# google/compare_gan

Hardware: NVIDIA H100
Metric: images/sec G+D step (resnet_cifar10) (higher is better)
Workload: dtype tf32

## Files before the change

### compare_gan_b200/_lib.py

```python
import ctypes
import os
import re

HERE = os.path.dirname(os.path.abspath(__file__))
HEADER = os.path.join(HERE, "..", "include", "cgan_b200.h")
SO_PATH = os.path.join(HERE, "csrc", "libcgan_b200.so")


class ConvDesc(ctypes.Structure):
  _fields_ = [(n, ctypes.c_int32) for n in
              ("n", "h", "w", "cin", "cout", "kh", "kw", "stride", "upsample", "oh", "ow", "pad_t", "pad_l")]


class ConvEpilogue(ctypes.Structure):
  _fields_ = [("bias", ctypes.c_void_p), ("residual", ctypes.c_void_p), ("mask", ctypes.c_void_p),
              ("mask_leak", ctypes.c_float), ("flags", ctypes.c_int32), ("ldy", ctypes.c_int32)]


CONV_RELU, CONV_ROUND_OUT, CONV_IN_TF32, CONV_IN2_TF32 = 1, 2, 4, 8
ACT_ROUND_TF32 = 0x100
OPT_TC_MT, OPT_LAST_PATH, OPT_TC_HALO, OPT_TC_THIN = 1, 2, 3, 6
OPT_LAST_TC_BN, OPT_LAST_TC_MT, OPT_LAST_TC_HALO, OPT_LAST_TC_CTAS_PER_SM, OPT_LAST_TC_EP_SMEM = 7, 8, 9, 10, 11
PATH_NAMES = {0: "simt_fp32", 1: "tcgen05_tf32", 2: "thin_fp32"}

_SCALARS = {"int": ctypes.c_int, "int32_t": ctypes.c_int32, "int64_t": ctypes.c_int64,
            "float": ctypes.c_float, "double": ctypes.c_double, "size_t": ctypes.c_size_t, "uint64_t": ctypes.c_uint64}


def parse_header(path=HEADER):
  src = open(path).read()
  src = re.sub(r"/\*.*?\*/", " ", src, flags=re.S)
  src = re.sub(r"//[^\n]*", " ", src)
  protos = {}
  for m in re.finditer(r"(const\s+char\s*\*|int64_t|int)\s+(cgan_\w+)\s*\(([^;{]*)\)\s*;", src):
    ret, name, args = m.group(1), m.group(2), m.group(3)
    restype = ctypes.c_char_p if "char" in ret else (ctypes.c_int64 if ret == "int64_t" else ctypes.c_int)
    argtypes = []
    args = args.strip()
    if args and args != "void":
      for a in args.split(","):
        a = a.strip()
        if "*" in a:
          argtypes.append(ctypes.c_void_p)
        else:
          ty = a.replace("const", "").split()[0]
          argtypes.append(_SCALARS[ty])
    protos[name] = (restype, argtypes)
  return protos


class CganError(RuntimeError):
  pass


_DLL = {}
# ... 65 lines not shown
```

### compare_gan_b200/csrc/common.cuh

```cuda
#pragma once
#include <cuda_runtime.h>
#include <stdint.h>
#include <stdio.h>
#include <string.h>

#include "../../include/cgan_b200.h"

struct cgan_ctx {
  int device;
  cudaStream_t stream;
  void* ws;
  size_t ws_bytes;
  int math_mode;
  int64_t launches;
  int num_sms;
  int tc_mt_max;
  int tc_halo;
  int tc_thin;
  int last_path;
  int last_tc_bn, last_tc_mt, last_tc_halo;
  int last_tc_ctas_per_sm;
  int last_tc_ep_smem;
  unsigned* counters;
  void* p2p;
  char err[512];
};

constexpr int CGAN_NUM_COUNTERS = 1 << 18;

static inline int cgan_fail(cgan_ctx* ctx, int code, const char* fmt, const char* a = "", const char* b = "") {
  if (ctx) snprintf(ctx->err, sizeof(ctx->err), fmt, a, b);
  return code;
}

#define CGAN_REQUIRE(ctx, cond, msg)                                              \
  do {                                                                            \
    if (!(cond)) return cgan_fail((ctx), CGAN_ERR_ARG, "%s: %s", __func__, msg);  \
  } while (0)

#define CGAN_CUDA(ctx, call)                                                                        \
  do {                                                                                              \
    cudaError_t e__ = (call);                                                                       \
    if (e__ != cudaSuccess) return cgan_fail((ctx), CGAN_ERR_CUDA, "%s: %s", __func__, cudaGetErrorString(e__)); \
  } while (0)

#define CGAN_LAUNCHED(ctx)                                                                          \
  do {                                                                                              \
    (ctx)->launches++;                                                                              \
    cudaError_t e__ = cudaGetLastError();                                                           \
    if (e__ != cudaSuccess) return cgan_fail((ctx), CGAN_ERR_CUDA, "%s: launch: %s", __func__, cudaGetErrorString(e__)); \
  } while (0)

static inline int cgan_ws(cgan_ctx* ctx, size_t bytes, void** out) {
  if (bytes > ctx->ws_bytes) {
    cudaStreamCaptureStatus st = cudaStreamCaptureStatusNone;
// ... 222 lines not shown
```

### compare_gan_b200/csrc/conv_tc.cu

```cuda
#include "tc_common.cuh"

namespace {

using namespace tc;

constexpr int TC_BM = 128;
constexpr int TC_BK = 32;
constexpr int TC_MAX_STAGES = 4;
constexpr int TC_MAX_TAPS = 32;
constexpr int TC_CWARPS = 8;
constexpr int TC_THREADS = 32 * TC_CWARPS + 32;
constexpr int TC_A_BYTES = TC_BM * TC_BK * 4;
constexpr int TC_WG_A_BYTES = TC_A_BYTES / 2;
constexpr int TC_ACC_COLS = 256;

struct TcParams {
  int ntaps, kchunks;
  int off_h[TC_MAX_TAPS], off_w[TC_MAX_TAPS], wtap[TC_MAX_TAPS], amap[TC_MAX_TAPS];
  int bw, bh, bni;
  int tiles_w, tiles_h;
  int rows_used;
  int img_n;
  int relu;
  int vec2;
  int round_a;
  int round_out;
  float mask_leak;
  const float* residual;
  const float* mask;
  int wimg_stride;
  int bn;
  int stages;
  int mt;
  int tiles_total;
  int cout;
  long long s_n, s_h, s_w, base;
  float* out;
  const float* bias;
  int nphases;
  int ph_tap0[5];
  long long ph_base[4];
  int ph_h[4], ph_w[4];
  int hg, hnv;
  int h_off_w[4], h_off_h0[4], h_wtap[4][4];
  int a_halo_bytes;
  int a_box_bytes;
  int sa_stages, sb_stages;
  int ep_smem;
};

struct AMaps { CUtensorMap m[4]; };


__device__ __forceinline__ void tc_tile_origin(const TcParams& p, int t, int& ow0, int& oh0, int& n0) {
  const int tw = t % p.tiles_w; t /= p.tiles_w;
  const int th = t % p.tiles_h;
  const int tn = t / p.tiles_h;
  ow0 = tw * p.bw; oh0 = th * p.bh; n0 = tn * p.bni;
}

__device__ __forceinline__ float epilogue_one(const TcParams& p, float v, int col, long long off) {
  if (p.bias) v += p.bias[col];
  if (p.residual) v += p.residual[off];
  if (p.relu) v = fmaxf(v, 0.f);
  if (p.mask) v = p.mask[off] > 0.f ? v : p.mask_leak * v;
  if (p.round_out) v = rna_tf32(v);
  return v;
}

template <int BN>
__device__ __forceinline__ void tile_epilogue(const TcParams& p, const float* acc, int tile, int nb0, int wg, int warp, int lane,
                                            long long out_base) {
  int ow0, oh0, n0;
  tc_tile_origin(p, tile, ow0, oh0, n0);
  const int c2 = (lane & 3) * 2;
#pragma unroll
  for (int h = 0; h < 2; ++h) {
    const int m = wg * 64 + (warp & 3) * 16 + (lane >> 2) + h * 8;
    const int wi = m % p.bw;
    const int hi = (m / p.bw) % p.bh;
    const int ni = m / (p.bw * p.bh);
    if (!(m < p.rows_used && n0 + ni < p.img_n && oh0 + hi < p.ph_h[blockIdx.z] && ow0 + wi < p.ph_w[blockIdx.z])) continue;
    const long long roff = out_base + (long long)(n0 + ni) * p.s_n + (long long)(oh0 + hi) * p.s_h +
                           (long long)(ow0 + wi) * p.s_w + nb0;
#pragma unroll
    for (int j = 0; j < BN / 8; ++j) {
      const int c = j * 8 + c2;
      if (nb0 + c >= p.cout) continue;
      float2 v = make_float2(acc[4 * j + 2 * h], acc[4 * j + 2 * h + 1]);
      const long long off = roff + c;
      if (p.vec2) {
        if (p.bias) { const float2 b = *reinterpret_cast<const float2*>(p.bias + nb0 + c); v.x += b.x; v.y += b.y; }
        if (p.residual) { const float2 r = *reinterpret_cast<const float2*>(p.residual + off); v.x += r.x; v.y += r.y; }
        if (p.relu) { v.x = fmaxf(v.x, 0.f); v.y = fmaxf(v.y, 0.f); }
        if (p.mask) {
          const float2 mv = *reinterpret_cast<const float2*>(p.mask + off);
          v.x = mv.x > 0.f ? v.x : p.mask_leak * v.x; v.y = mv.y > 0.f ? v.y : p.mask_leak * v.y;
        }
        if (p.round_out) { v.x = rna_tf32(v.x); v.y = rna_tf32(v.y); }
        *reinterpret_cast<float2*>(p.out + off) = v;
      } else {
        p.out[off] = epilogue_one(p, v.x, nb0 + c, off);
        if (nb0 + c + 1 < p.cout) p.out[off + 1] = epilogue_one(p, v.y, nb0 + c + 1, off + 1);
      }
    }
  }
}

template <int BN>
__device__ __forceinline__ void tile_epilogue_smem(const TcParams& p, const float* acc, int tile, int nb0, int wg, int warp,
                                                 int lane, long long out_base, const uint8_t* smem, int stage_bytes,
                                                 uint64_t* full_bar, uint64_t* empty_bar, int& stage, uint32_t& phase,
                                                 int& chunk, int chunks, const float* s_bias) {
  int ow0, oh0, n0;
  tc_tile_origin(p, tile, ow0, oh0, n0);
  const int c2 = (lane & 3) * 2;
  bool ok[2];
  long long roff[2];
  int m[2];
#pragma unroll
  for (int h = 0; h < 2; ++h) {
    m[h] = wg * 64 + (warp & 3) * 16 + (lane >> 2) + h * 8;
    const int wi = m[h] % p.bw;
    const int hi = (m[h] / p.bw) % p.bh;
    const int ni = m[h] / (p.bw * p.bh);
    ok[h] = m[h] < p.rows_used && n0 + ni < p.img_n && oh0 + hi < p.ph_h[blockIdx.z] && ow0 + wi < p.ph_w[blockIdx.z];
    roff[h] = out_base + (long long)(n0 + ni) * p.s_n + (long long)(oh0 + hi) * p.s_h + (long long)(ow0 + wi) * p.s_w + nb0;
  }
  const uint32_t bias_addr = smem_u32(s_bias);
#pragma unroll
  for (int cc = 0; cc < BN / 32; ++cc) {
    mbar_wait(&full_bar[stage], phase);
    const uint32_t e_addr = smem_u32(smem + stage * stage_bytes);
#pragma unroll
    for (int jj = 0; jj < 4; ++jj) {
      const int j = cc * 4 + jj, c = j * 8 + c2;
      if (nb0 + c >= p.cout) continue;
      const float2 b = p.bias ? lds64(bias_addr + c * 4) : make_float2(0.f, 0.f);
#pragma unroll
      for (int h = 0; h < 2; ++h) {
        if (!ok[h]) continue;
        float2 v = make_float2(acc[4 * j + 2 * h], acc[4 * j + 2 * h + 1]);
        const float2 e = lds64(e_addr + sw128_offset(m[h], jj * 8 + c2));
        if (p.bias) { v.x += b.x; v.y += b.y; }
        if (p.residual) { v.x += e.x; v.y += e.y; }
        if (p.relu) { v.x = fmaxf(v.x, 0.f); v.y = fmaxf(v.y, 0.f); }
        if (p.mask) { v.x = e.x > 0.f ? v.x : p.mask_leak * v.x; v.y = e.y > 0.f ? v.y : p.mask_leak * v.y; }
        if (p.round_out) { v.x = rna_tf32(v.x); v.y = rna_tf32(v.y); }
        *reinterpret_cast<float2*>(p.out + roff[h] + c) = v;
      }
    }
    if (chunk + p.stages < chunks) {
      fence_proxy_async();
      named_bar(1 + wg, 128);
      if ((threadIdx.x & 127) == 0) mbar_arrive(&empty_bar[stage]);
    }
    ++chunk;
    if (++stage == p.stages) { stage = 0; phase ^= 1; }
  }
}

constexpr int tc_min_ctas(int bn, int mt) { return bn * mt <= 128 ? 2 : 1; }

__device__ __forceinline__ void tc_round_smem(uint32_t base, int bytes, int q, int nthreads) {
#pragma unroll 4
  for (int i = q * 16; i < bytes; i += nthreads * 16) {
    float4 v = lds128(base + i);
    v.x = rna_tf32(v.x); v.y = rna_tf32(v.y); v.z = rna_tf32(v.z); v.w = rna_tf32(v.w);
    sts128(base + i, v);
  }
}

template <int BN, int MT>
__global__ void __launch_bounds__(TC_THREADS, tc_min_ctas(BN, MT))
conv_tc_kernel(const __grid_constant__ AMaps tm_as, const __grid_constant__ CUtensorMap tm_b, const TcParams p,
               const __grid_constant__ AMaps tm_e) {
  extern __shared__ __align__(1024) uint8_t smem_raw[];
  uint8_t* smem = reinterpret_cast<uint8_t*>((reinterpret_cast<uintptr_t>(smem_raw) + 1023) & ~uintptr_t(1023));
  constexpr int b_bytes = BN * TC_BK * 4;
  constexpr int a_bytes = MT * TC_A_BYTES;
  constexpr int stage_bytes = a_bytes + b_bytes;
  uint64_t* full_bar = reinterpret_cast<uint64_t*>(smem + p.stages * stage_bytes);
  uint64_t* empty_bar = full_bar + p.stages;
  float* s_bias = reinterpret_cast<float*>(smem + p.stages * stage_bytes + 256);

  const int warp = threadIdx.x >> 5, lane = threadIdx.x & 31;
  const int tap0 = p.ph_tap0[blockIdx.z];
  const int num_kb = (p.ph_tap0[blockIdx.z + 1] - tap0) * p.kchunks;

  const int tile0 = blockIdx.x * MT;
  const int nt_here = max(0, min(MT, p.tiles_total - tile0));
  const int nb0 = blockIdx.y * BN;

  if (threadIdx.x == 0) {
    for (int s = 0; s < p.stages; ++s) {
      mbar_init(&full_bar[s], 1);
      mbar_init(&empty_bar[s], 2);
    }
    asm volatile("fence.mbarrier_init.release.cluster;" ::: "memory");
  }
  __syncthreads();

  if (warp == TC_CWARPS) {
    if (lane == 0) {
      asm volatile("prefetch.tensormap [%0];" ::"l"(&tm_as.m[0]) : "memory");
      asm volatile("prefetch.tensormap [%0];" ::"l"(&tm_b) : "memory");
      int stage = 0;
      uint32_t phase = 0;
      for (int kb = 0; kb < num_kb; ++kb) {
        const int tl = kb / p.kchunks, kc = kb - tl * p.kchunks, tap = tap0 + tl;
        mbar_wait(&empty_bar[stage], phase ^ 1);
        uint8_t* sa = smem + stage * stage_bytes;
        uint8_t* sb = sa + a_bytes;
        mbar_expect_tx(&full_bar[stage], (uint32_t)(nt_here * p.rows_used * TC_BK * 4 + b_bytes));
        int ow0, oh0, n0;
        for (int i = 0; i < nt_here; ++i) {
          tc_tile_origin(p, tile0 + i, ow0, oh0, n0);
          tma_load_4d(sa + i * TC_A_BYTES, &tm_as.m[p.amap[tap]], &full_bar[stage], kc * TC_BK, ow0 + p.off_w[tap],
                      oh0 + p.off_h[tap], n0);
        }
        tc_tile_origin(p, tile0, ow0, oh0, n0);
        tma_load_3d(sb, &tm_b, &full_bar[stage], kc * TC_BK, nb0, p.wtap[tap] + n0 * p.wimg_stride);
        if (++stage == p.stages) { stage = 0; phase ^= 1; }
      }
      if (p.ep_smem) {
        const CUtensorMap* em = &tm_e.m[blockIdx.z];
        for (int t = 0; t < nt_here; ++t) {
          int ow0, oh0, n0;
          tc_tile_origin(p, tile0 + t, ow0, oh0, n0);
          for (int cc = 0; cc < BN / 32; ++cc) {
            mbar_wait(&empty_bar[stage], phase ^ 1);
            mbar_expect_tx(&full_bar[stage], (uint32_t)(p.rows_used * TC_BK * 4));
            tma_load_4d(smem + stage * stage_bytes, em, &full_bar[stage], nb0 + cc * 32, ow0, oh0, n0);
            if (++stage == p.stages) { stage = 0; phase ^= 1; }
          }
        }
      }
    }
  } else {
    const int wg = warp >> 2;
    const int q = threadIdx.x & 127;
    if (p.ep_smem && p.bias)
      for (int i = threadIdx.x; i < BN; i += 32 * TC_CWARPS) s_bias[i] = nb0 + i < p.cout ? p.bias[nb0 + i] : 0.f;
    float acc[MT][BN / 2];
#pragma unroll
    for (int t = 0; t < MT; ++t)
#pragma unroll
      for (int i = 0; i < BN / 2; ++i) acc[t][i] = 0.f;
    int stage = 0, prev = -1;
    uint32_t phase = 0;
    for (int kb = 0; kb < num_kb; ++kb) {
      mbar_wait(&full_bar[stage], phase);
      const uint32_t a_addr = smem_u32(smem + stage * stage_bytes) + wg * TC_WG_A_BYTES;
      const uint32_t b_addr = smem_u32(smem + stage * stage_bytes) + a_bytes;
      if (p.round_a) {
        for (int tl = 0; tl < nt_here; ++tl) tc_round_smem(a_addr + tl * TC_A_BYTES, TC_WG_A_BYTES, q, 128);
        fence_proxy_async();
        named_bar(1 + wg, 128);
      }
#pragma unroll
      for (int t = 0; t < MT; ++t)
#pragma unroll
        for (int i = 0; i < BN / 2; ++i) acc_fence(acc[t][i]);
      wgmma_fence();
#pragma unroll
      for (int t = 0; t < MT; ++t) {
#pragma unroll
        for (int k = 0; k < TC_BK / 8; ++k)
          wgmma_tf32<BN>(acc[t], make_desc(a_addr + t * TC_A_BYTES + k * 32), make_desc(b_addr + k * 32));
      }
      wgmma_commit();
      wgmma_wait<1>();
#pragma unroll
      for (int t = 0; t < MT; ++t)
#pragma unroll
        for (int i = 0; i < BN / 2; ++i) acc_fence(acc[t][i]);
      if (prev >= 0 && q == 0) mbar_arrive(&empty_bar[prev]);
      prev = stage;
      if (++stage == p.stages) { stage = 0; phase ^= 1; }
    }
    wgmma_wait<0>();
    if (p.ep_smem) {
      if (prev >= 0 && q == 0) mbar_arrive(&empty_bar[prev]);
      named_bar(3, 32 * TC_CWARPS);
      int chunk = 0;
#pragma unroll
      for (int t = 0; t < MT; ++t) {
#pragma unroll
        for (int i = 0; i < BN / 2; ++i) acc_fence(acc[t][i]);
        if (t < nt_here)
          tile_epilogue_smem<BN>(p, acc[t], tile0 + t, nb0, wg, warp, lane, p.ph_base[blockIdx.z], smem, stage_bytes,
                                 full_bar, empty_bar, stage, phase, chunk, nt_here * (BN / 32), s_bias);
      }
    } else {
#pragma unroll
      for (int t = 0; t < MT; ++t) {
#pragma unroll
        for (int i = 0; i < BN / 2; ++i) acc_fence(acc[t][i]);
        if (t < nt_here) tile_epilogue<BN>(p, acc[t], tile0 + t, nb0, wg, warp, lane, p.ph_base[blockIdx.z]);
      }
    }
  }
}

template <int BN, int MT>
__global__ void __launch_bounds__(TC_THREADS, 1)
conv_tc_halo_kernel(const __grid_constant__ CUtensorMap tm_a, const __grid_constant__ CUtensorMap tm_b, const TcParams p) {
  extern __shared__ __align__(1024) uint8_t smem_raw[];
  uint8_t* smem = reinterpret_cast<uint8_t*>((reinterpret_cast<uintptr_t>(smem_raw) + 1023) & ~uintptr_t(1023));
  constexpr int b_bytes = BN * TC_BK * 4;
  const int a_stage = MT * p.a_halo_bytes;
  uint8_t* smem_b = smem + p.sa_stages * a_stage;
  uint64_t* a_full = reinterpret_cast<uint64_t*>(smem_b + p.sb_stages * b_bytes);
  uint64_t* a_empty = a_full + p.sa_stages;
  uint64_t* b_full = a_empty + p.sa_stages;
  uint64_t* b_empty = b_full + p.sb_stages;

  const int warp = threadIdx.x >> 5, lane = threadIdx.x & 31;
  const int tile0 = blockIdx.x * MT;
  const int nt_here = min(MT, p.tiles_total - tile0);
  const int nb0 = blockIdx.y * BN;

  if (threadIdx.x == 0) {
    for (int s = 0; s < p.sa_stages; ++s) {
      mbar_init(&a_full[s], 1);
      mbar_init(&a_empty[s], 2);
// ... 132 lines not shown
  int best = tc_pick_bn(ncols_pad);
  if (best == 0 || tiles_m * (ncols_pad / best) >= sms) return best;
  int pick = best;
  for (int b = best - 32; b >= 64; b -= 32) {
    if (ncols_pad % b) continue;
    pick = b;
    if (tiles_m * (ncols_pad / b) >= sms) break;
  }
  return pick;
}

constexpr int TC_NARROW_WAVES = 2;
constexpr int TC_NARROW_MAX_KB = 96;

inline int tc_pick_bn_per_tap(int ncols_pad, long long tiles_m, const TcParams& p, int sms) {
  const int bn = tc_pick_bn_occupancy(ncols_pad, tiles_m, sms);
  int kb = 0;
  for (int i = 0; i < p.nphases; ++i) {
    const int k = (p.ph_tap0[i + 1] - p.ph_tap0[i]) * p.kchunks;
    if (k > kb) kb = k;
  }
  if (bn == 256 && tiles_m * (ncols_pad / 256) * p.nphases >= (long long)TC_NARROW_WAVES * sms && kb <= TC_NARROW_MAX_KB)
    return 128;
  return bn;
}


inline int tc_vec2(const TcParams& p) {
  long long odd = p.cout | p.s_n | p.s_h | p.s_w | p.base;
  for (int i = 0; i < p.nphases; ++i) odd |= p.ph_base[i];
  return (odd & 1) ? 0 : 1;
}

inline bool tc_ep_smem_ok(const TcParams& p, const TcConv& c) {
  const float* e = c.residual ? c.residual : c.mask;
  if (!e || (c.residual && c.mask) || !p.vec2 || (reinterpret_cast<uintptr_t>(e) & 15)) return false;
  long long a = p.s_n | p.s_h | p.s_w;
  for (int i = 0; i < p.nphases; ++i) a |= p.ph_base[i];
  return (a & 3) == 0;
}

int prep_weights(cgan_ctx* ctx, const TcConv& c, int kdim_pad, int ncols_pad, float** out) {
  void* ws = nullptr;
  int rc = cgan_ws(ctx, (size_t)c.taps_total * ncols_pad * kdim_pad * sizeof(float), &ws);
  if (rc) return rc;
  float* wt = reinterpret_cast<float*>(ws);
  long long tot = (long long)c.taps_total * ncols_pad * kdim_pad;
  long long blocks = (tot + 255) / 256, cap = (long long)ctx->num_sms * 8;
  wprep_kernel<<<(int)(blocks > cap ? cap : blocks), 256, 0, ctx->stream>>>(wt, c.wsrc, c.taps_total, c.ncols, ncols_pad, c.a.ch,
                                                                             kdim_pad, c.transpose_w);
  CGAN_LAUNCHED(ctx);
  *out = wt;
  return CGAN_OK;
}

bool make_weight_map(CUtensorMap* tm, float* wt, int kdim_pad, int ncols_pad, int taps_total, int bn) {
  cuuint64_t dims[3] = {(cuuint64_t)kdim_pad, (cuuint64_t)ncols_pad, (cuuint64_t)taps_total};
  cuuint64_t strides[2] = {(cuuint64_t)kdim_pad * 4, (cuuint64_t)ncols_pad * kdim_pad * 4};
  cuuint32_t box[3] = {TC_BK, (cuuint32_t)bn, 1};
  cuuint32_t es[3] = {1, 1, 1};
  return get_encode()(tm, CU_TENSOR_MAP_DATA_TYPE_FLOAT32, 3, wt, dims, strides, box, es, CU_TENSOR_MAP_INTERLEAVE_NONE,
                      CU_TENSOR_MAP_SWIZZLE_128B, CU_TENSOR_MAP_L2_PROMOTION_L2_256B,
                      CU_TENSOR_MAP_FLOAT_OOB_FILL_NONE) == CUDA_SUCCESS;
}

template <typename Kernel>
int tc_ctas_per_sm(Kernel kernel, size_t smem) {
  int blocks = 0;
  if (cudaOccupancyMaxActiveBlocksPerMultiprocessor(&blocks, kernel, TC_THREADS, smem) != cudaSuccess) blocks = 0;
  return blocks;
}

template <int BN, int MT>
int tc_launch_t(cgan_ctx* ctx, bool halo, dim3 grid, size_t smem, const AMaps& as, const CUtensorMap& b, const TcParams& p,
                const AMaps& es) {
  static bool attr_set[2] = {false, false};
  if (halo) {
    if (!attr_set[1]) {
      CGAN_CUDA(ctx, cudaFuncSetAttribute(conv_tc_halo_kernel<BN, MT>, cudaFuncAttributeMaxDynamicSharedMemorySize, 227 * 1024));
      attr_set[1] = true;
    }
    ctx->last_tc_ctas_per_sm = tc_ctas_per_sm(conv_tc_halo_kernel<BN, MT>, smem);
    conv_tc_halo_kernel<BN, MT><<<grid, TC_THREADS, smem, ctx->stream>>>(as.m[0], b, p);
  } else {
    if (!attr_set[0]) {
      CGAN_CUDA(ctx, cudaFuncSetAttribute(conv_tc_kernel<BN, MT>, cudaFuncAttributeMaxDynamicSharedMemorySize, 227 * 1024));
      attr_set[0] = true;
    }
    ctx->last_tc_ctas_per_sm = tc_ctas_per_sm(conv_tc_kernel<BN, MT>, smem);
    conv_tc_kernel<BN, MT><<<grid, TC_THREADS, smem, ctx->stream>>>(as, b, p, es);
  }
  CGAN_LAUNCHED(ctx);
  return CGAN_OK;
}

int tc_launch(cgan_ctx* ctx, bool halo, dim3 grid, size_t smem, const AMaps& as, const CUtensorMap& b, const TcParams& p,
              const AMaps& es) {
  ctx->last_tc_bn = p.bn; ctx->last_tc_mt = p.mt; ctx->last_tc_halo = halo ? 1 : 0; ctx->last_tc_ep_smem = p.ep_smem;
#define TC_CASE(BN, MT) \
  if (p.bn == BN && p.mt == MT) return tc_launch_t<BN, MT>(ctx, halo, grid, smem, as, b, p, es);
  TC_CASE(32, 1) TC_CASE(64, 1) TC_CASE(96, 1) TC_CASE(128, 1) TC_CASE(160, 1) TC_CASE(192, 1) TC_CASE(224, 1)
  TC_CASE(256, 1) TC_CASE(32, 2) TC_CASE(64, 2) TC_CASE(96, 2) TC_CASE(128, 2)
#undef TC_CASE
  return cgan_fail(ctx, CGAN_ERR_UNSUPPORTED, "%s: no kernel for this column tile / pixel-tile count%s", "cgan_conv_tc");
}

}

bool cgan_tc_shape_ok(int n, int h, int w, int kdim, int ncols) {
  if (n < 1 || h < 1 || w < 1 || ncols < 1) return false;
  if (kdim < 8 || kdim % 4 != 0) return false;
  if (ncols > 256 && ncols % 32 != 0) return false;
  int bn = tc_pick_bn((ncols + 31) / 32 * 32);
  return bn != 0 && bn % 32 == 0;
}

int cgan_conv_tc(cgan_ctx* ctx, const TcConv& c) {
  if (!get_encode()) return cgan_fail(ctx, CGAN_ERR_UNSUPPORTED, "%s: cuTensorMapEncodeTiled unavailable%s", "cgan_conv_tc");
  const ConvTaps& tp = c.taps;
  if (tp.ntaps > TC_MAX_TAPS || c.a.nviews > 4) return cgan_fail(ctx, CGAN_ERR_UNSUPPORTED, "%s: too many taps/views%s", "cgan_conv_tc");
  const int n = c.a.n, h = c.a.h, w = c.a.w, kdim = c.a.ch, gh = c.gh, gw = c.gw, ntaps = tp.ntaps;
  TcParams p;
  memset(&p, 0, sizeof(p));
  p.ntaps = ntaps;
  const int kdim_pad = (kdim + TC_BK - 1) / TC_BK * TC_BK;
  p.kchunks = kdim_pad / TC_BK;
  for (int i = 0; i < ntaps; ++i) {
    p.off_h[i] = tp.off_h[i]; p.off_w[i] = tp.off_w[i]; p.wtap[i] = tp.wtap[i]; p.amap[i] = tp.view[i];
  }
  int tiles_n;
  tc_geometry(n, gh, gw, &p.bw, &p.bh, &p.bni, &p.tiles_w, &p.tiles_h, &tiles_n);
  p.rows_used = p.bw * p.bh * p.bni;
  p.img_n = n;
// ... 63 lines not shown
      p.tiles_w = w / hbw; p.tiles_h = h / hbh;
      const long long tiles_total = (long long)p.tiles_w * p.tiles_h * n;
      p.rows_used = 128;
      p.bn = tc_pick_bn_occupancy(ncols_pad, tiles_total, ctx->num_sms);
      const int ncol_tiles = ncols_pad / p.bn;
      p.a_box_bytes = (hbh + 2) * hbw * 128;
      p.a_halo_bytes = (p.a_box_bytes + 1023) / 1024 * 1024;
      const int b_bytes = p.bn * TC_BK * 4;
      const int budget = 227 * 1024 - 1024 - 512;
      const int mt_cap = ctx->tc_mt_max >= 2 ? 2 : 1;
      p.sa_stages = 2;
      p.mt = 1;
      for (int m = mt_cap; m >= 2; --m) {
        if (m * p.bn > TC_ACC_COLS || tiles_total * ncol_tiles < 2ll * m * ctx->num_sms) continue;
        if ((budget - p.sa_stages * m * p.a_halo_bytes) / b_bytes < 4) continue;
        p.mt = m;
        break;
      }
      p.sb_stages = (budget - p.sa_stages * p.mt * p.a_halo_bytes) / b_bytes;
      if (p.sb_stages > 8) p.sb_stages = 8;
      ok = p.sb_stages >= 2;
      if (ok) {
        p.tiles_total = (int)tiles_total;
        AMaps tm_a;
        CUtensorMap tm_b;
        memset(&tm_a, 0, sizeof(tm_a));
        if (!make_act_map(&tm_a.m[0], c.a.in + c.a.view_off[0], kdim, w, h, n, c.a.sw, c.a.sh, c.a.sn, hbw, hbh + 2, 1))
          return cgan_fail(ctx, CGAN_ERR_CUDA, "%s: cuTensorMapEncodeTiled(A halo) failed%s", "cgan_conv_tc");
        if (!make_weight_map(&tm_b, wt, kdim_pad, ncols_pad, c.taps_total, p.bn))
          return cgan_fail(ctx, CGAN_ERR_CUDA, "%s: cuTensorMapEncodeTiled(B) failed%s", "cgan_conv_tc");
        p.vec2 = tc_vec2(p);
        size_t smem = (size_t)p.sa_stages * p.mt * p.a_halo_bytes + (size_t)p.sb_stages * b_bytes + 1024 + 512;
        dim3 grid((unsigned)((tiles_total + p.mt - 1) / p.mt), (unsigned)ncol_tiles);
        return tc_launch(ctx, true, grid, smem, tm_a, tm_b, p, tm_a);
      }
    }
    tc_geometry(n, gh, gw, &p.bw, &p.bh, &p.bni, &p.tiles_w, &p.tiles_h, &tiles_n);
    p.rows_used = p.bw * p.bh * p.bni;
    p.bn = tc_pick_bn_per_tap(ncols_pad, (long long)p.tiles_w * p.tiles_h * tiles_n, p, ctx->num_sms);
    p.hg = p.hnv = 0;
  }

  AMaps tm_as;
  CUtensorMap tm_b;
  memset(&tm_as, 0, sizeof(tm_as));
  for (int v = 0; v < 4; ++v)
    if (!make_view_map(&tm_as.m[v], c.a, v, p.bw, p.bh, p.bni))
      return cgan_fail(ctx, CGAN_ERR_CUDA, "%s: cuTensorMapEncodeTiled(A) failed%s", "cgan_conv_tc");
  if (!make_weight_map(&tm_b, wt, kdim_pad, ncols_pad, c.taps_total, p.bn))
    return cgan_fail(ctx, CGAN_ERR_CUDA, "%s: cuTensorMapEncodeTiled(B) failed%s", "cgan_conv_tc");

  const long long tiles_total = (long long)p.tiles_w * p.tiles_h * tiles_n;
  const int ncol_tiles = ncols_pad / p.bn;
  p.tiles_total = (int)tiles_total;
  p.mt = 1;
  if (ctx->tc_mt_max >= 2 && 2 * p.bn <= 128 && tiles_total * ncol_tiles * p.nphases >= 4ll * ctx->num_sms &&
      (c.wimg_stride == 0 || (p.tiles_w * p.tiles_h) % 2 == 0))
    p.mt = 2;
  const bool two_ctas = p.mt * p.bn <= 128;
  const size_t stage_bytes = (size_t)p.mt * TC_A_BYTES + (size_t)p.bn * TC_BK * 4;
  p.stages = (int)(((two_ctas ? 110 : 220) * 1024) / stage_bytes);
  if (p.stages > TC_MAX_STAGES) p.stages = TC_MAX_STAGES;
  if (p.stages < 2) p.stages = 2;
  p.vec2 = tc_vec2(p);
  AMaps tm_e;
  memset(&tm_e, 0, sizeof(tm_e));
  p.ep_smem = tc_ep_smem_ok(p, c) ? 1 : 0;
  for (int v = 0; p.ep_smem && v < p.nphases; ++v)
    if (!make_act_map(&tm_e.m[v], (c.residual ? c.residual : c.mask) + p.ph_base[v], c.ncols, p.ph_w[v], p.ph_h[v], n,
                      p.s_w, p.s_h, p.s_n, p.bw, p.bh, p.bni))
      return cgan_fail(ctx, CGAN_ERR_CUDA, "%s: cuTensorMapEncodeTiled(residual / mask) failed%s", "cgan_conv_tc");
  size_t smem = (size_t)p.stages * stage_bytes + 1024  + 256  + (p.ep_smem ? p.bn * 4 : 0) ;
  dim3 grid((unsigned)((tiles_total + p.mt - 1) / p.mt), (unsigned)ncol_tiles, (unsigned)p.nphases);
  return tc_launch(ctx, false, grid, smem, tm_as, tm_b, p, tm_e);
}
```

### compare_gan_b200/csrc/pointwise.cu

```cuda
#include "common.cuh"

int cgan_version(void) { return 1; }

int cgan_ctx_create(cgan_ctx** out, int device) {
  if (!out) return CGAN_ERR_ARG;
  *out = nullptr;
  int count = 0;
  if (cudaGetDeviceCount(&count) != cudaSuccess || device < 0 || device >= count) return CGAN_ERR_CUDA;
  cgan_ctx* c = new cgan_ctx();
  memset(c, 0, sizeof(*c));
  c->device = device;
  if (cudaSetDevice(device) != cudaSuccess) { delete c; return CGAN_ERR_CUDA; }
  cudaDeviceProp prop;
  if (cudaGetDeviceProperties(&prop, device) != cudaSuccess) { delete c; return CGAN_ERR_CUDA; }
  c->num_sms = prop.multiProcessorCount;
  c->tc_mt_max = 2;
  if (const char* e = getenv("CGAN_TC_MT")) c->tc_mt_max = atoi(e) >= 2 ? 2 : 1;
  c->tc_halo = 1;
  if (const char* e = getenv("CGAN_TC_HALO")) c->tc_halo = atoi(e) ? 1 : 0;
  c->tc_thin = 1;
  if (const char* e = getenv("CGAN_TC_THIN")) c->tc_thin = atoi(e) ? 1 : 0;
  c->stream = 0;
  if (cudaMalloc(reinterpret_cast<void**>(&c->counters), CGAN_NUM_COUNTERS * sizeof(unsigned)) != cudaSuccess ||
      cudaMemset(c->counters, 0, CGAN_NUM_COUNTERS * sizeof(unsigned)) != cudaSuccess) {
// ... 34 lines not shown
int cgan_ctx_set_option(cgan_ctx* ctx, int key, int64_t value) {
  if (!ctx) return CGAN_ERR_ARG;
  switch (key) {
    case CGAN_OPT_TC_MT:
      CGAN_REQUIRE(ctx, value == 1 || value == 2, "CGAN_OPT_TC_MT must be 1 or 2");
      ctx->tc_mt_max = (int)value;
      return CGAN_OK;
    case CGAN_OPT_TC_HALO:
      CGAN_REQUIRE(ctx, value >= 0 && value <= 2, "CGAN_OPT_TC_HALO must be 0, 1 or 2");
      ctx->tc_halo = (int)value;
      return CGAN_OK;
    case CGAN_OPT_TC_THIN:
      CGAN_REQUIRE(ctx, value == 0 || value == 1, "CGAN_OPT_TC_THIN must be 0 or 1");
      ctx->tc_thin = (int)value;
      return CGAN_OK;
    default:
      return cgan_fail(ctx, CGAN_ERR_ARG, "%s: unknown or read-only option%s", "cgan_ctx_set_option");
  }
}

int cgan_ctx_get_option(cgan_ctx* ctx, int key, int64_t* host_value) {
  if (!ctx) return CGAN_ERR_ARG;
  CGAN_REQUIRE(ctx, host_value, "null pointer");
  switch (key) {
    case CGAN_OPT_TC_MT: *host_value = ctx->tc_mt_max; return CGAN_OK;
    case CGAN_OPT_LAST_PATH: *host_value = ctx->last_path; return CGAN_OK;
    case CGAN_OPT_TC_HALO: *host_value = ctx->tc_halo; return CGAN_OK;
    case CGAN_OPT_TC_THIN: *host_value = ctx->tc_thin; return CGAN_OK;
    case CGAN_OPT_LAST_TC_BN: *host_value = ctx->last_tc_bn; return CGAN_OK;
    case CGAN_OPT_LAST_TC_MT: *host_value = ctx->last_tc_mt; return CGAN_OK;
    case CGAN_OPT_LAST_TC_HALO: *host_value = ctx->last_tc_halo; return CGAN_OK;
    case CGAN_OPT_LAST_TC_CTAS_PER_SM: *host_value = ctx->last_tc_ctas_per_sm; return CGAN_OK;
    case CGAN_OPT_LAST_TC_EP_SMEM: *host_value = ctx->last_tc_ep_smem; return CGAN_OK;
    default:
      return cgan_fail(ctx, CGAN_ERR_ARG, "%s: unknown option%s", "cgan_ctx_get_option");
  }
}

const char* cgan_last_error(cgan_ctx* ctx) { return ctx ? ctx->err : "null context"; }
int64_t cgan_launch_count(cgan_ctx* ctx) { return ctx ? ctx->launches : -1; }

namespace {

#define EW_LOOP(i, n)                                                                  \
  for (long long i = (long long)blockIdx.x * blockDim.x + threadIdx.x, s__ = (long long)gridDim.x * blockDim.x; \
       i < (n); i += s__)

__global__ void fill_kernel(float* d, float v, long long n) { EW_LOOP(i, n) d[i] = v; }
__global__ void copy_kernel(float* __restrict__ d, const float* __restrict__ s, long long n) { EW_LOOP(i, n) d[i] = s[i]; }
__global__ void copy2d_kernel(float* __restrict__ d, int dld, int doff, const float* __restrict__ s, int sld, int soff,
                              long long rows, int cols) {
  long long n = rows * cols;
  EW_LOOP(i, n) {
    long long r = i / cols;
    int j = (int)(i % cols);
    d[r * dld + doff + j] = s[r * sld + soff + j];
  }
}
__global__ void axpby_kernel(float* __restrict__ y, float a, const float* __restrict__ x, float b,
                             const float* __restrict__ y0, float c, long long n) {
  EW_LOOP(i, n) {
    float v = a * x[i] + c;
    if (y0) v += b * y0[i];
    y[i] = v;
  }
}
// ... 810 lines not shown
```

### compare_gan_b200/csrc/tc_common.cuh

```cuda
#pragma once
#include <cuda.h>

#include "common.cuh"
#include "wgmma_tf32.cuh"

namespace tc {

__device__ __forceinline__ uint32_t smem_u32(const void* p) { return (uint32_t)__cvta_generic_to_shared(p); }

__device__ __forceinline__ void mbar_init(uint64_t* bar, uint32_t count) {
  asm volatile("mbarrier.init.shared::cta.b64 [%0], %1;" ::"r"(smem_u32(bar)), "r"(count));
}
__device__ __forceinline__ void mbar_expect_tx(uint64_t* bar, uint32_t bytes) {
  asm volatile("mbarrier.arrive.expect_tx.shared::cta.b64 _, [%0], %1;" ::"r"(smem_u32(bar)), "r"(bytes) : "memory");
}
__device__ __forceinline__ void mbar_arrive(uint64_t* bar) {
  asm volatile("mbarrier.arrive.shared::cta.b64 _, [%0];" ::"r"(smem_u32(bar)) : "memory");
}
__device__ __forceinline__ void mbar_wait(uint64_t* bar, uint32_t parity) {
  uint32_t addr = smem_u32(bar);
  asm volatile(
      "{\n\t"
      ".reg .pred p;\n\t"
      "WAIT_LOOP:\n\t"
      "mbarrier.try_wait.parity.shared::cta.b64 p, [%0], %1;\n\t"
      "@p bra WAIT_DONE;\n\t"
      "bra WAIT_LOOP;\n\t"
      "WAIT_DONE:\n\t"
      "}\n" ::"r"(addr), "r"(parity) : "memory");
}

__device__ __forceinline__ void tma_load_4d(void* dst, const CUtensorMap* map, uint64_t* bar, int c0, int c1, int c2, int c3) {
  asm volatile(
      "cp.async.bulk.tensor.4d.shared::cluster.global.tile.mbarrier::complete_tx::bytes [%0], [%1, {%3, %4, %5, %6}], [%2];"
      ::"r"(smem_u32(dst)), "l"(map), "r"(smem_u32(bar)), "r"(c0), "r"(c1), "r"(c2), "r"(c3) : "memory");
}
__device__ __forceinline__ void tma_load_3d(void* dst, const CUtensorMap* map, uint64_t* bar, int c0, int c1, int c2) {
  asm volatile(
      "cp.async.bulk.tensor.3d.shared::cluster.global.tile.mbarrier::complete_tx::bytes [%0], [%1, {%3, %4, %5}], [%2];"
      ::"r"(smem_u32(dst)), "l"(map), "r"(smem_u32(bar)), "r"(c0), "r"(c1), "r"(c2) : "memory");
}

__device__ __forceinline__ uint64_t make_desc(uint32_t smem_addr) {
  uint64_t d = 0;
  d |= (uint64_t)((smem_addr & 0x3FFFF) >> 4);
  d |= (uint64_t)1 << 16;
  d |= (uint64_t)(1024 >> 4) << 32;
  d |= (uint64_t)1 << 62;
  return d;
}

__device__ __forceinline__ void wgmma_fence() { asm volatile("wgmma.fence.sync.aligned;" ::: "memory"); }
__device__ __forceinline__ void wgmma_commit() { asm volatile("wgmma.commit_group.sync.aligned;" ::: "memory"); }
template <int N>
__device__ __forceinline__ void wgmma_wait() { asm volatile("wgmma.wait_group.sync.aligned %0;" ::"n"(N) : "memory"); }
__device__ __forceinline__ void acc_fence(float& r) { asm volatile("" : "+f"(r)::"memory"); }
__device__ __forceinline__ void named_bar(int id, int count) { asm volatile("bar.sync %0, %1;" ::"r"(id), "r"(count) : "memory"); }
__device__ __forceinline__ void fence_proxy_async() { asm volatile("fence.proxy.async.shared::cta;" ::: "memory"); }

__device__ __forceinline__ uint32_t sw128_offset(int row, int k) {
  return (uint32_t)(row * 128 + ((((k >> 2) ^ row) & 7) << 4) + (k & 3) * 4);
}

__device__ __forceinline__ float4 lds128(uint32_t addr) {
  float4 v;
  asm volatile("ld.shared.v4.f32 {%0, %1, %2, %3}, [%4];" : "=f"(v.x), "=f"(v.y), "=f"(v.z), "=f"(v.w) : "r"(addr));
  return v;
}
__device__ __forceinline__ float2 lds64(uint32_t addr) {
  float2 v;
  asm volatile("ld.shared.v2.f32 {%0, %1}, [%2];" : "=f"(v.x), "=f"(v.y) : "r"(addr));
  return v;
}
__device__ __forceinline__ float lds32(uint32_t addr) {
  float v;
  asm volatile("ld.shared.f32 %0, [%1];" : "=f"(v) : "r"(addr));
  return v;
}
__device__ __forceinline__ void sts128(uint32_t addr, float4 v) {
  asm volatile("st.shared.v4.f32 [%0], {%1, %2, %3, %4};" ::"r"(addr), "f"(v.x), "f"(v.y), "f"(v.z), "f"(v.w) : "memory");
}

typedef CUresult (*EncodeTiledFn)(CUtensorMap*, CUtensorMapDataType, cuuint32_t, void*, const cuuint64_t*, const cuuint64_t*,
                                  const cuuint32_t*, const cuuint32_t*, CUtensorMapInterleave, CUtensorMapSwizzle,
                                  CUtensorMapL2promotion, CUtensorMapFloatOOBfill);

inline EncodeTiledFn get_encode() {
  static EncodeTiledFn fn = nullptr;
  if (!fn) {
    void* p = nullptr;
    cudaDriverEntryPointQueryResult q;
    if (cudaGetDriverEntryPoint("cuTensorMapEncodeTiled", &p, cudaEnableDefault, &q) == cudaSuccess &&
        q == cudaDriverEntryPointSuccess)
      fn = reinterpret_cast<EncodeTiledFn>(p);
  }
  return fn;
}


inline bool make_act_map(CUtensorMap* tm, const float* base, int c, int w, int h, int n, long long sw, long long sh,
                         long long sn, int bw, int bh, int bni, CUtensorMapSwizzle swizzle = CU_TENSOR_MAP_SWIZZLE_128B) {
  EncodeTiledFn enc = get_encode();
  if (!enc) return false;
  cuuint64_t dims[4] = {(cuuint64_t)c, (cuuint64_t)w, (cuuint64_t)h, (cuuint64_t)n};
  cuuint64_t strides[3] = {(cuuint64_t)sw * 4, (cuuint64_t)sh * 4, (cuuint64_t)sn * 4};
  cuuint32_t box[4] = {32, (cuuint32_t)bw, (cuuint32_t)bh, (cuuint32_t)bni};
  cuuint32_t es[4] = {1, 1, 1, 1};
  return enc(tm, CU_TENSOR_MAP_DATA_TYPE_FLOAT32, 4, const_cast<float*>(base), dims, strides, box, es,
             CU_TENSOR_MAP_INTERLEAVE_NONE, swizzle, CU_TENSOR_MAP_L2_PROMOTION_L2_128B,
             CU_TENSOR_MAP_FLOAT_OOB_FILL_NONE) == CUDA_SUCCESS;
// ... 13 lines not shown
```

### include/cgan_b200.h

```cpp
#ifndef CGAN_B200_H_
#define CGAN_B200_H_

#include <stddef.h>
#include <stdint.h>

#ifdef __cplusplus
extern "C" {
#endif

typedef struct cgan_ctx cgan_ctx;

enum { CGAN_OK = 0, CGAN_ERR_ARG = 1, CGAN_ERR_CUDA = 2, CGAN_ERR_WORKSPACE = 3, CGAN_ERR_UNSUPPORTED = 4 };

int cgan_version(void);
int cgan_ctx_create(cgan_ctx** out, int device);
int cgan_ctx_destroy(cgan_ctx* ctx);
int cgan_ctx_set_stream(cgan_ctx* ctx, void* cuda_stream);
int cgan_ctx_reserve_workspace(cgan_ctx* ctx, size_t bytes);
int cgan_ctx_set_math_mode(cgan_ctx* ctx, int mode);
const char* cgan_last_error(cgan_ctx* ctx);
int64_t cgan_launch_count(cgan_ctx* ctx);
enum { CGAN_OPT_TC_MT = 1, CGAN_OPT_LAST_PATH = 2, CGAN_OPT_TC_HALO = 3, CGAN_OPT_TC_THIN = 6, CGAN_OPT_LAST_TC_BN = 7,
       CGAN_OPT_LAST_TC_MT = 8, CGAN_OPT_LAST_TC_HALO = 9, CGAN_OPT_LAST_TC_CTAS_PER_SM = 10,
       CGAN_OPT_LAST_TC_EP_SMEM = 11 };
enum { CGAN_PATH_SIMT_FP32 = 0, CGAN_PATH_TCGEN05_TF32 = 1, CGAN_PATH_THIN_FP32 = 2 };
int cgan_ctx_set_option(cgan_ctx* ctx, int key, int64_t value);
int cgan_ctx_get_option(cgan_ctx* ctx, int key, int64_t* host_value);

int cgan_fill(cgan_ctx*, float* dst, float value, int64_t n);
int cgan_copy(cgan_ctx*, float* dst, const float* src, int64_t n);
int cgan_copy2d(cgan_ctx*, float* dst, int dst_ld, int dst_off, const float* src, int src_ld, int src_off,
                int64_t rows, int cols);
int cgan_axpby(cgan_ctx*, float* y, float a, const float* x, float b, const float* y0, float c, int64_t n);
int cgan_scale_by_dev(cgan_ctx*, float* y, const float* x, const float* scalar_dev, float mul, int inverse, int64_t n);
int cgan_dot(cgan_ctx*, float* out_dev, const float* a, const float* b, int64_t n);
int cgan_random_uniform(cgan_ctx*, float* out, int64_t n, uint64_t seed, uint64_t offset);
int cgan_interpolate(cgan_ctx*, float* y, const float* x, const float* xf, const float* alpha, int n, int64_t per);
int cgan_one_hot(cgan_ctx*, float* out, const int32_t* labels, int n, int classes);

typedef struct {
  int32_t n, h, w, cin;
  int32_t cout, kh, kw, stride;
  int32_t upsample;
  int32_t oh, ow;
  int32_t pad_t, pad_l;
} cgan_conv_desc;

int cgan_conv2d_fwd(cgan_ctx*, const cgan_conv_desc*, const float* x, const float* w_hwio, const float* bias, float* y);
int cgan_conv2d_fwd_act(cgan_ctx*, const cgan_conv_desc*, const float* x, const float* w_hwio, const float* bias, int act,
                        float* y);
int cgan_conv2d_fwd_act_ld(cgan_ctx*, const cgan_conv_desc*, const float* x, const float* w_hwio, const float* bias, int act,
                           float* y, int ldy);
int cgan_conv2d_dgrad(cgan_ctx*, const cgan_conv_desc*, const float* dy, const float* w_hwio, float* dx);
int cgan_conv2d_wgrad(cgan_ctx*, const cgan_conv_desc*, const float* x, const float* dy, float* dw);
enum { CGAN_CONV_RELU = 1, CGAN_CONV_ROUND_OUT = 2, CGAN_CONV_IN_TF32 = 4, CGAN_CONV_IN2_TF32 = 8 };
typedef struct {
  const float* bias;
// ... 196 lines not shown
```

Baseline: 21570.

## Store conv epilogue output through shared memory with TMA bulk tensor stores

The tensor-core conv epilogue now writes the biased, activated results into swizzled shared-memory stage buffers and has one thread issue 4D TMA stores to global memory, replacing per-thread scattered float2 global stores. The path is enabled for all aligned vec2 convs, not only those with a residual or mask operand. The producer warp just signals full barriers when there is no operand to load, and stage release is delayed until the bulk store has finished reading the buffer. This adds a CTA-wide named barrier per 32-column chunk and a serial wait on bulk-store reads, which could stall the pipeline.

```diff
diff --git a/compare_gan_b200/_lib.py b/compare_gan_b200/_lib.py
--- a/compare_gan_b200/_lib.py
+++ b/compare_gan_b200/_lib.py
@@ -21,6 +21,7 @@
 ACT_ROUND_TF32 = 0x100
 OPT_TC_MT, OPT_LAST_PATH, OPT_TC_HALO, OPT_TC_THIN = 1, 2, 3, 6
 OPT_LAST_TC_BN, OPT_LAST_TC_MT, OPT_LAST_TC_HALO, OPT_LAST_TC_CTAS_PER_SM, OPT_LAST_TC_EP_SMEM = 7, 8, 9, 10, 11
+OPT_LAST_TC_TMA_STORE = 12
 PATH_NAMES = {0: "simt_fp32", 1: "tcgen05_tf32", 2: "thin_fp32"}
 
 _SCALARS = {"int": ctypes.c_int, "int32_t": ctypes.c_int32, "int64_t": ctypes.c_int64,
diff --git a/compare_gan_b200/csrc/common.cuh b/compare_gan_b200/csrc/common.cuh
--- a/compare_gan_b200/csrc/common.cuh
+++ b/compare_gan_b200/csrc/common.cuh
@@ -21,6 +21,7 @@
   int last_tc_bn, last_tc_mt, last_tc_halo;
   int last_tc_ctas_per_sm;
   int last_tc_ep_smem;
+  int last_tc_tma_store;
   unsigned* counters;
   void* p2p;
   char err[512];
diff --git a/compare_gan_b200/csrc/conv_tc.cu b/compare_gan_b200/csrc/conv_tc.cu
--- a/compare_gan_b200/csrc/conv_tc.cu
+++ b/compare_gan_b200/csrc/conv_tc.cu
@@ -46,6 +46,7 @@
   int a_halo_bytes;
   int a_box_bytes;
   int sa_stages, sb_stages;
+  int ep_tma;
   int ep_smem;
 };
 
@@ -108,26 +109,15 @@
 }
 
 template <int BN>
-__device__ __forceinline__ void tile_epilogue_smem(const TcParams& p, const float* acc, int tile, int nb0, int wg, int warp,
-                                                 int lane, long long out_base, const uint8_t* smem, int stage_bytes,
+__device__ __forceinline__ void tile_epilogue_smem(const TcParams& p, const CUtensorMap* om, const float* acc, int tile,
+                                                 int nb0, int wg, int warp, int lane, const uint8_t* smem, int stage_bytes,
                                                  uint64_t* full_bar, uint64_t* empty_bar, int& stage, uint32_t& phase,
-                                                 int& chunk, int chunks, const float* s_bias) {
+                                                 int& chunk, int chunks, uint32_t bias_addr) {
   int ow0, oh0, n0;
   tc_tile_origin(p, tile, ow0, oh0, n0);
   const int c2 = (lane & 3) * 2;
-  bool ok[2];
-  long long roff[2];
-  int m[2];
-#pragma unroll
-  for (int h = 0; h < 2; ++h) {
-    m[h] = wg * 64 + (warp & 3) * 16 + (lane >> 2) + h * 8;
-    const int wi = m[h] % p.bw;
-    const int hi = (m[h] / p.bw) % p.bh;
-    const int ni = m[h] / (p.bw * p.bh);
-    ok[h] = m[h] < p.rows_used && n0 + ni < p.img_n && oh0 + hi < p.ph_h[blockIdx.z] && ow0 + wi < p.ph_w[blockIdx.z];
-    roff[h] = out_base + (long long)(n0 + ni) * p.s_n + (long long)(oh0 + hi) * p.s_h + (long long)(ow0 + wi) * p.s_w + nb0;
-  }
-  const uint32_t bias_addr = smem_u32(s_bias);
+  const int m0 = wg * 64 + (warp & 3) * 16 + (lane >> 2);
+  const bool operand = p.residual || p.mask;
 #pragma unroll
   for (int cc = 0; cc < BN / 32; ++cc) {
     mbar_wait(&full_bar[stage], phase);
@@ -135,25 +125,27 @@
 #pragma unroll
     for (int jj = 0; jj < 4; ++jj) {
       const int j = cc * 4 + jj, c = j * 8 + c2;
-      if (nb0 + c >= p.cout) continue;
       const float2 b = p.bias ? lds64(bias_addr + c * 4) : make_float2(0.f, 0.f);
 #pragma unroll
       for (int h = 0; h < 2; ++h) {
-        if (!ok[h]) continue;
+        const uint32_t a = e_addr + sw128_offset(m0 + h * 8, jj * 8 + c2);
         float2 v = make_float2(acc[4 * j + 2 * h], acc[4 * j + 2 * h + 1]);
-        const float2 e = lds64(e_addr + sw128_offset(m[h], jj * 8 + c2));
+        const float2 e = operand ? lds64(a) : make_float2(0.f, 0.f);
         if (p.bias) { v.x += b.x; v.y += b.y; }
         if (p.residual) { v.x += e.x; v.y += e.y; }
         if (p.relu) { v.x = fmaxf(v.x, 0.f); v.y = fmaxf(v.y, 0.f); }
         if (p.mask) { v.x = e.x > 0.f ? v.x : p.mask_leak * v.x; v.y = e.y > 0.f ? v.y : p.mask_leak * v.y; }
         if (p.round_out) { v.x = rna_tf32(v.x); v.y = rna_tf32(v.y); }
-        *reinterpret_cast<float2*>(p.out + roff[h] + c) = v;
-      }
-    }
-    if (chunk + p.stages < chunks) {
-      fence_proxy_async();
-      named_bar(1 + wg, 128);
-      if ((threadIdx.x & 127) == 0) mbar_arrive(&empty_bar[stage]);
+        sts64(a, v);
+      }
+    }
+    fence_proxy_async();
+    named_bar(3, 32 * TC_CWARPS);
+    if (threadIdx.x == 0) {
+      tma_store_4d(om, e_addr, nb0 + cc * 32, ow0, oh0, n0);
+      bulk_commit();
+      bulk_wait_read<1>();
+      if (chunk >= 1 && chunk - 1 + p.stages < chunks) mbar_arrive(&empty_bar[stage == 0 ? p.stages - 1 : stage - 1], 2);
     }
     ++chunk;
     if (++stage == p.stages) { stage = 0; phase ^= 1; }
@@ -174,7 +166,7 @@
 template <int BN, int MT>
 __global__ void __launch_bounds__(TC_THREADS, tc_min_ctas(BN, MT))
 conv_tc_kernel(const __grid_constant__ AMaps tm_as, const __grid_constant__ CUtensorMap tm_b, const TcParams p,
-               const __grid_constant__ AMaps tm_e) {
+               const __grid_constant__ AMaps tm_e, const __grid_constant__ AMaps tm_o) {
   extern __shared__ __align__(1024) uint8_t smem_raw[];
   uint8_t* smem = reinterpret_cast<uint8_t*>((reinterpret_cast<uintptr_t>(smem_raw) + 1023) & ~uintptr_t(1023));
   constexpr int b_bytes = BN * TC_BK * 4;
@@ -223,15 +215,19 @@
         tma_load_3d(sb, &tm_b, &full_bar[stage], kc * TC_BK, nb0, p.wtap[tap] + n0 * p.wimg_stride);
         if (++stage == p.stages) { stage = 0; phase ^= 1; }
       }
-      if (p.ep_smem) {
+      if (p.ep_tma) {
         const CUtensorMap* em = &tm_e.m[blockIdx.z];
         for (int t = 0; t < nt_here; ++t) {
           int ow0, oh0, n0;
           tc_tile_origin(p, tile0 + t, ow0, oh0, n0);
           for (int cc = 0; cc < BN / 32; ++cc) {
             mbar_wait(&empty_bar[stage], phase ^ 1);
-            mbar_expect_tx(&full_bar[stage], (uint32_t)(p.rows_used * TC_BK * 4));
-            tma_load_4d(smem + stage * stage_bytes, em, &full_bar[stage], nb0 + cc * 32, ow0, oh0, n0);
+            if (p.ep_smem) {
+              mbar_expect_tx(&full_bar[stage], (uint32_t)(p.rows_used * TC_BK * 4));
+              tma_load_4d(smem + stage * stage_bytes, em, &full_bar[stage], nb0 + cc * 32, ow0, oh0, n0);
+            } else {
+              mbar_arrive(&full_bar[stage]);
+            }
             if (++stage == p.stages) { stage = 0; phase ^= 1; }
           }
         }
@@ -240,7 +236,7 @@
   } else {
     const int wg = warp >> 2;
     const int q = threadIdx.x & 127;
-    if (p.ep_smem && p.bias)
+    if (p.ep_tma && p.bias)
       for (int i = threadIdx.x; i < BN; i += 32 * TC_CWARPS) s_bias[i] = nb0 + i < p.cout ? p.bias[nb0 + i] : 0.f;
     float acc[MT][BN / 2];
 #pragma unroll
@@ -280,7 +276,7 @@
       if (++stage == p.stages) { stage = 0; phase ^= 1; }
     }
     wgmma_wait<0>();
-    if (p.ep_smem) {
+    if (p.ep_tma) {
       if (prev >= 0 && q == 0) mbar_arrive(&empty_bar[prev]);
       named_bar(3, 32 * TC_CWARPS);
       int chunk = 0;
@@ -289,9 +285,10 @@
 #pragma unroll
         for (int i = 0; i < BN / 2; ++i) acc_fence(acc[t][i]);
         if (t < nt_here)
-          tile_epilogue_smem<BN>(p, acc[t], tile0 + t, nb0, wg, warp, lane, p.ph_base[blockIdx.z], smem, stage_bytes,
-                                 full_bar, empty_bar, stage, phase, chunk, nt_here * (BN / 32), s_bias);
-      }
+          tile_epilogue_smem<BN>(p, &tm_o.m[blockIdx.z], acc[t], tile0 + t, nb0, wg, warp, lane, smem, stage_bytes,
+                                 full_bar, empty_bar, stage, phase, chunk, nt_here * (BN / 32), smem_u32(s_bias));
+      }
+      if (threadIdx.x == 0) bulk_wait_read<0>();
     } else {
 #pragma unroll
       for (int t = 0; t < MT; ++t) {
@@ -490,13 +487,16 @@
   return (odd & 1) ? 0 : 1;
 }
 
-inline bool tc_ep_smem_ok(const TcParams& p, const TcConv& c) {
+inline bool tc_ep_tma_ok(const TcParams& p, const TcConv& c) {
   const float* e = c.residual ? c.residual : c.mask;
-  if (!e || (c.residual && c.mask) || !p.vec2 || (reinterpret_cast<uintptr_t>(e) & 15)) return false;
+  if (!p.vec2 || (c.residual && c.mask) || ((reinterpret_cast<uintptr_t>(c.out) | reinterpret_cast<uintptr_t>(e)) & 15))
+    return false;
   long long a = p.s_n | p.s_h | p.s_w;
   for (int i = 0; i < p.nphases; ++i) a |= p.ph_base[i];
   return (a & 3) == 0;
 }
+
+static_assert(3 * sizeof(AMaps) + sizeof(CUtensorMap) + sizeof(TcParams) + 2 * 63 <= 4096, "conv_tc_kernel parameters");
 
 int prep_weights(cgan_ctx* ctx, const TcConv& c, int kdim_pad, int ncols_pad, float** out) {
   void* ws = nullptr;
@@ -531,7 +531,7 @@
 
 template <int BN, int MT>
 int tc_launch_t(cgan_ctx* ctx, bool halo, dim3 grid, size_t smem, const AMaps& as, const CUtensorMap& b, const TcParams& p,
-                const AMaps& es) {
+                const AMaps& es, const AMaps& os) {
   static bool attr_set[2] = {false, false};
   if (halo) {
     if (!attr_set[1]) {
@@ -546,17 +546,18 @@
       attr_set[0] = true;
     }
     ctx->last_tc_ctas_per_sm = tc_ctas_per_sm(conv_tc_kernel<BN, MT>, smem);
-    conv_tc_kernel<BN, MT><<<grid, TC_THREADS, smem, ctx->stream>>>(as, b, p, es);
+    conv_tc_kernel<BN, MT><<<grid, TC_THREADS, smem, ctx->stream>>>(as, b, p, es, os);
   }
   CGAN_LAUNCHED(ctx);
   return CGAN_OK;
 }
 
 int tc_launch(cgan_ctx* ctx, bool halo, dim3 grid, size_t smem, const AMaps& as, const CUtensorMap& b, const TcParams& p,
-              const AMaps& es) {
+              const AMaps& es, const AMaps& os) {
   ctx->last_tc_bn = p.bn; ctx->last_tc_mt = p.mt; ctx->last_tc_halo = halo ? 1 : 0; ctx->last_tc_ep_smem = p.ep_smem;
+  ctx->last_tc_tma_store = p.ep_tma;
 #define TC_CASE(BN, MT) \
-  if (p.bn == BN && p.mt == MT) return tc_launch_t<BN, MT>(ctx, halo, grid, smem, as, b, p, es);
+  if (p.bn == BN && p.mt == MT) return tc_launch_t<BN, MT>(ctx, halo, grid, smem, as, b, p, es, os);
   TC_CASE(32, 1) TC_CASE(64, 1) TC_CASE(96, 1) TC_CASE(128, 1) TC_CASE(160, 1) TC_CASE(192, 1) TC_CASE(224, 1)
   TC_CASE(256, 1) TC_CASE(32, 2) TC_CASE(64, 2) TC_CASE(96, 2) TC_CASE(128, 2)
 #undef TC_CASE
@@ -686,7 +687,7 @@
         p.vec2 = tc_vec2(p);
         size_t smem = (size_t)p.sa_stages * p.mt * p.a_halo_bytes + (size_t)p.sb_stages * b_bytes + 1024 + 512;
         dim3 grid((unsigned)((tiles_total + p.mt - 1) / p.mt), (unsigned)ncol_tiles);
-        return tc_launch(ctx, true, grid, smem, tm_a, tm_b, p, tm_a);
+        return tc_launch(ctx, true, grid, smem, tm_a, tm_b, p, tm_a, tm_a);
       }
     }
     tc_geometry(n, gh, gw, &p.bw, &p.bh, &p.bni, &p.tiles_w, &p.tiles_h, &tiles_n);
@@ -717,14 +718,20 @@
   if (p.stages > TC_MAX_STAGES) p.stages = TC_MAX_STAGES;
   if (p.stages < 2) p.stages = 2;
   p.vec2 = tc_vec2(p);
-  AMaps tm_e;
+  AMaps tm_e, tm_o;
   memset(&tm_e, 0, sizeof(tm_e));
-  p.ep_smem = tc_ep_smem_ok(p, c) ? 1 : 0;
-  for (int v = 0; p.ep_smem && v < p.nphases; ++v)
-    if (!make_act_map(&tm_e.m[v], (c.residual ? c.residual : c.mask) + p.ph_base[v], c.ncols, p.ph_w[v], p.ph_h[v], n,
-                      p.s_w, p.s_h, p.s_n, p.bw, p.bh, p.bni))
+  memset(&tm_o, 0, sizeof(tm_o));
+  p.ep_tma = tc_ep_tma_ok(p, c) ? 1 : 0;
+  p.ep_smem = p.ep_tma && (c.residual || c.mask) ? 1 : 0;
+  for (int v = 0; p.ep_tma && v < p.nphases; ++v) {
+    if (!make_act_map(&tm_o.m[v], c.out + p.ph_base[v], c.ncols, p.ph_w[v], p.ph_h[v], n, p.s_w, p.s_h, p.s_n, p.bw, p.bh,
+                      p.bni))
+      return cgan_fail(ctx, CGAN_ERR_CUDA, "%s: cuTensorMapEncodeTiled(output) failed%s", "cgan_conv_tc");
+    if (p.ep_smem && !make_act_map(&tm_e.m[v], (c.residual ? c.residual : c.mask) + p.ph_base[v], c.ncols, p.ph_w[v],
+                                   p.ph_h[v], n, p.s_w, p.s_h, p.s_n, p.bw, p.bh, p.bni))
       return cgan_fail(ctx, CGAN_ERR_CUDA, "%s: cuTensorMapEncodeTiled(residual / mask) failed%s", "cgan_conv_tc");
-  size_t smem = (size_t)p.stages * stage_bytes + 1024  + 256  + (p.ep_smem ? p.bn * 4 : 0) ;
+  }
+  size_t smem = (size_t)p.stages * stage_bytes + 1024  + 256  + (p.ep_tma ? p.bn * 4 : 0) ;
   dim3 grid((unsigned)((tiles_total + p.mt - 1) / p.mt), (unsigned)ncol_tiles, (unsigned)p.nphases);
-  return tc_launch(ctx, false, grid, smem, tm_as, tm_b, p, tm_e);
-}
+  return tc_launch(ctx, false, grid, smem, tm_as, tm_b, p, tm_e, tm_o);
+}
diff --git a/compare_gan_b200/csrc/pointwise.cu b/compare_gan_b200/csrc/pointwise.cu
--- a/compare_gan_b200/csrc/pointwise.cu
+++ b/compare_gan_b200/csrc/pointwise.cu
@@ -90,6 +90,7 @@
     case CGAN_OPT_LAST_TC_HALO: *host_value = ctx->last_tc_halo; return CGAN_OK;
     case CGAN_OPT_LAST_TC_CTAS_PER_SM: *host_value = ctx->last_tc_ctas_per_sm; return CGAN_OK;
     case CGAN_OPT_LAST_TC_EP_SMEM: *host_value = ctx->last_tc_ep_smem; return CGAN_OK;
+    case CGAN_OPT_LAST_TC_TMA_STORE: *host_value = ctx->last_tc_tma_store; return CGAN_OK;
     default:
       return cgan_fail(ctx, CGAN_ERR_ARG, "%s: unknown option%s", "cgan_ctx_get_option");
   }
diff --git a/compare_gan_b200/csrc/tc_common.cuh b/compare_gan_b200/csrc/tc_common.cuh
--- a/compare_gan_b200/csrc/tc_common.cuh
+++ b/compare_gan_b200/csrc/tc_common.cuh
@@ -16,6 +16,9 @@
 }
 __device__ __forceinline__ void mbar_arrive(uint64_t* bar) {
   asm volatile("mbarrier.arrive.shared::cta.b64 _, [%0];" ::"r"(smem_u32(bar)) : "memory");
+}
+__device__ __forceinline__ void mbar_arrive(uint64_t* bar, uint32_t count) {
+  asm volatile("mbarrier.arrive.shared::cta.b64 _, [%0], %1;" ::"r"(smem_u32(bar)), "r"(count) : "memory");
 }
 __device__ __forceinline__ void mbar_wait(uint64_t* bar, uint32_t parity) {
   uint32_t addr = smem_u32(bar);
@@ -40,6 +43,13 @@
       "cp.async.bulk.tensor.3d.shared::cluster.global.tile.mbarrier::complete_tx::bytes [%0], [%1, {%3, %4, %5}], [%2];"
       ::"r"(smem_u32(dst)), "l"(map), "r"(smem_u32(bar)), "r"(c0), "r"(c1), "r"(c2) : "memory");
 }
+__device__ __forceinline__ void tma_store_4d(const CUtensorMap* map, uint32_t src, int c0, int c1, int c2, int c3) {
+  asm volatile("cp.async.bulk.tensor.4d.global.shared::cta.bulk_group [%0, {%2, %3, %4, %5}], [%1];"
+               ::"l"(map), "r"(src), "r"(c0), "r"(c1), "r"(c2), "r"(c3) : "memory");
+}
+__device__ __forceinline__ void bulk_commit() { asm volatile("cp.async.bulk.commit_group;" ::: "memory"); }
+template <int N>
+__device__ __forceinline__ void bulk_wait_read() { asm volatile("cp.async.bulk.wait_group.read %0;" ::"n"(N) : "memory"); }
 
 __device__ __forceinline__ uint64_t make_desc(uint32_t smem_addr) {
   uint64_t d = 0;
@@ -76,6 +86,9 @@
   float v;
   asm volatile("ld.shared.f32 %0, [%1];" : "=f"(v) : "r"(addr));
   return v;
+}
+__device__ __forceinline__ void sts64(uint32_t addr, float2 v) {
+  asm volatile("st.shared.v2.f32 [%0], {%1, %2};" ::"r"(addr), "f"(v.x), "f"(v.y) : "memory");
 }
 __device__ __forceinline__ void sts128(uint32_t addr, float4 v) {
   asm volatile("st.shared.v4.f32 [%0], {%1, %2, %3, %4};" ::"r"(addr), "f"(v.x), "f"(v.y), "f"(v.z), "f"(v.w) : "memory");
diff --git a/include/cgan_b200.h b/include/cgan_b200.h
--- a/include/cgan_b200.h
+++ b/include/cgan_b200.h
@@ -22,7 +22,7 @@
 int64_t cgan_launch_count(cgan_ctx* ctx);
 enum { CGAN_OPT_TC_MT = 1, CGAN_OPT_LAST_PATH = 2, CGAN_OPT_TC_HALO = 3, CGAN_OPT_TC_THIN = 6, CGAN_OPT_LAST_TC_BN = 7,
        CGAN_OPT_LAST_TC_MT = 8, CGAN_OPT_LAST_TC_HALO = 9, CGAN_OPT_LAST_TC_CTAS_PER_SM = 10,
-       CGAN_OPT_LAST_TC_EP_SMEM = 11 };
+       CGAN_OPT_LAST_TC_EP_SMEM = 11, CGAN_OPT_LAST_TC_TMA_STORE = 12 };
 enum { CGAN_PATH_SIMT_FP32 = 0, CGAN_PATH_TCGEN05_TF32 = 1, CGAN_PATH_THIN_FP32 = 2 };
 int cgan_ctx_set_option(cgan_ctx* ctx, int key, int64_t value);
 int cgan_ctx_get_option(cgan_ctx* ctx, int key, int64_t* host_value);
```

Result: faster. 22980, median of 6 (+6.5%).
